# xxayt/MGSV

Measured on AMD Instinct MI355X. Metric: video-music pairs/s fwd+bwd at B=64 (full training step); sub-objects: retrieval sim-matrix GB/s, eval forward pairs/s, higher is better.
Workload: dtype bf16; 1 GPU; BASELINE.json configs[2]: B=64/GPU, T_v=30, T_a=512, D=512, train mode (dropout on), f32 master weights + Adam, f32 gradient accumulation; global_batch=64, launch=tape

## Files before the change

### include/made_hip.h

```cpp
#ifndef MADE_HIP_H
#define MADE_HIP_H

#include <stdint.h>

#ifdef __cplusplus
extern "C" {
#endif

#define MADE_ABI_VERSION 8

enum MadeDtype { MADE_F32 = 0, MADE_BF16 = 1 };

enum MadeAct {
    MADE_ACT_NONE = 0,
    MADE_ACT_RELU = 1,
    MADE_ACT_GELU = 2,
    MADE_ACT_QUICKGELU = 3,
    MADE_ACT_SIGMOID = 4
};

enum MadeGate {
    MADE_GATE_NONE = 0,
    MADE_GATE_RELU_OUT = 1,
    MADE_GATE_GELU_Z = 2,
// ... 629 lines not shown
} MadeResampleDesc;

int made_audio_resample(const float* pcm, int64_t pcm_len, const MadeResampleDesc* desc, int64_t n_tracks, const float* taps,
                        int64_t n_taps, float* out, int64_t out_len, void* stream);

typedef struct MadeAudioSegDesc {
    int64_t first;
    int64_t count;
} MadeAudioSegDesc;

int made_audio_fbank(const float* pcm, int64_t pcm_len, const MadeAudioSegDesc* segs, int64_t n_segs, const float* window,
                     const float* twiddle, const float* mel, int32_t mel_ld, float* spec, void* stream);

int made_ast_patches(const float* spec, int64_t n_segs, void* patches, int32_t patch_dtype, int64_t ld_patch, void* stream);

#ifdef __cplusplus
}
#endif
#endif
```

### mgsv_amd/_lib.py

```python
from __future__ import annotations

import ctypes as C
import os

_HERE = os.path.dirname(os.path.abspath(__file__))


def variant_env(name: str, default: str = "") -> str:
    if os.environ.get("MADE_DEBUG_VARIANTS", "0") in ("", "0"):
        return default
    return os.environ.get(name, default)


LIB_PATH = os.environ.get("MADE_LIB_PATH") or os.path.join(_HERE, "libmade_hip.so")
ABI_VERSION = 8

F32, BF16 = 0, 1
ACT_NONE, ACT_RELU, ACT_GELU, ACT_QUICKGELU, ACT_SIGMOID = 0, 1, 2, 3, 4
GATE_NONE, GATE_RELU_OUT, GATE_GELU_Z, GATE_QUICKGELU_Z, GATE_SIGMOID_OUT = 0, 1, 2, 3, 4

vp, i64, i32, f32 = C.c_void_p, C.c_int64, C.c_int32, C.c_float

WIDE_PLAN_HEAD, WIDE_PLAN_SAMPLE, WIDE_PLAN_SLOT, WIDE_PLAN_SLOT_BITS = 4, 4, 16, 8

# ... 169 lines not shown
                ("dtype", i32), ("_pad", i32)]


class MadeFrameDesc(C.Structure):
    _fields_ = [("offset", i64), ("coef", i64), ("H", i32), ("W", i32), ("kh", i32), ("kv", i32)]


class MadeResampleDesc(C.Structure):
    _fields_ = [("offset", i64), ("n", i64), ("taps", i64), ("o", i32), ("m", i32), ("width", i32), ("_pad", i32)]


class MadeAudioSegDesc(C.Structure):
    _fields_ = [("first", i64), ("count", i64)]


SIGNATURES = {
    "made_abi_version": (C.c_int, []),
    "made_set_f32_products": (C.c_int, [C.c_int]),
    "made_get_f32_products": (C.c_int, []),
    "made_last_error": (C.c_char_p, []),
    "made_device_info": (C.c_int, [C.c_char_p, C.c_int, C.POINTER(C.c_int), C.POINTER(C.c_int)]),
    "made_tape_begin": (C.c_int, []),
    "made_tape_end": (C.c_int, [C.POINTER(C.c_uint64)]),
    "made_tape_replay": (C.c_int, [C.c_uint64]),
    "made_tape_free": (C.c_int, [C.c_uint64]),
    "made_tape_interleave": (C.c_int, [C.c_uint64, i32]),
    "made_tape_count": (C.c_int, [C.c_uint64, C.POINTER(i64), C.POINTER(i64), C.POINTER(i64)]),
    "made_tape_replay_range": (C.c_int, [C.c_uint64, i64, i64]),
    "made_tape_op": (C.c_int, [C.c_uint64, i64, C.POINTER(i32), C.POINTER(C.c_uint64), C.POINTER(C.c_uint64), C.POINTER(C.c_uint32)]),
    "made_stream_wait": (C.c_int, [vp, vp]),
    "made_tape_event": (C.c_int, [i32, i32, vp]),
# ... 150 lines not shown
```

### mgsv_amd/ops_train.py

```python
from __future__ import annotations

import ctypes as C
from typing import Optional, Tuple

import torch

from . import _lib
from ._lib import BF16, F32, MadeAttnBwdArgs, MadeDropout, MadeGemmTNArgs, MadeGemmTNGroup, check, lib
from .ops import _f32, _p, _stream, _timed, dt_of, set_drop

Tensor = torch.Tensor
Pair = Tuple[int, int]


_TN_WS_LIMIT = 1 << 32
_TN_SLAB_US = 1.3


def _tn_splits(tiles: int, nslab: int, gathered: bool, cap: int) -> int:
    if _lib.variant_env("MADE_TN_SPLIT_MODEL", "1") == "0":
        sp = max(8, (512 // max(tiles, 1)) // 8 * 8) if cap == 64 and tiles < 64 else max(1, 2048 // max(tiles, 1))
        while (nslab + sp - 1) // sp > 64:
            sp += 8
        return min(sp, max(1, nslab))
    live = max(1, (nslab * 9) // 16 if gathered else nslab)
    best, best_t = 1, float("inf")
    for sp in (1, 2, 3, 4, 6, 8, 16, 24, 32, 40, 48, 56, 64):
# ... 242 lines not shown
    check(lib().made_pool_bwd(_p(_f32(mean, "mean")), _p(_f32(dvec, "dvec")), _p(_f32(mask, "mask")),
                              _p(in1), _dt(in1), *bs(in1), _p(in2), _dt(in2), *bs(in2),
                              _p(out), dt_of(out), *bs(out), B, T, D, eps, _stream()), "made_pool_bwd")
    return out


def l2norm_bwd(x: Tensor, dy: Tensor, dx: Optional[Tensor] = None, *, accumulate: bool = False, dx_alt: Optional[Tensor] = None,
               eps: float = 1e-12, dy_rows_per: int = 1) -> None:
    rows, D = x.shape
    check(lib().made_l2norm_bwd(_p(x), dt_of(x), x.stride(0), _p(_f32(dy, "dy")), dy.stride(0), dy_rows_per,
                                _p(dx), dx.stride(0) if dx is not None else 0, int(accumulate),
                                _p(dx_alt), _dt(dx_alt), dx_alt.stride(0) if dx_alt is not None else 0,
                                rows, D, eps, _stream()), "made_l2norm_bwd")


def clip_loss_bwd(sims: Tensor, logit_scale: Tensor, weight: float, upstream: Optional[Tensor], lse_ws: Tensor, dsims: Tensor,
                  dsims_t: Optional[Tensor], d_logit_scale: Optional[Tensor], accumulate: bool = False,
                  row_exclude: Optional[Tensor] = None) -> None:
    n = sims.shape[0]
    assert lse_ws.numel() >= 2 * n and dsims.is_contiguous()
    assert row_exclude is None or (row_exclude.shape == sims.shape and row_exclude.is_contiguous())
    check(lib().made_clip_loss_bwd(_p(_f32(sims, "sims")), sims.stride(0), n, _p(logit_scale), float(weight), _p(upstream),
                                   _p(lse_ws), _p(dsims), _p(dsims_t), int(accumulate), _p(d_logit_scale),
                                   _p(_f32(row_exclude, "row_exclude")), _stream()),
          "made_clip_loss_bwd")


def xpool_tail_bwd(y: Tensor, gamma: Tensor, beta: Tensor, video: Tensor, dsims: Tensor, dy: Tensor, Nm: int, Nv: int, *,
                   dy_drop: Optional[Tensor] = None, drop=None, dgamma: Optional[Tensor] = None, dbeta: Optional[Tensor] = None,
                   dvideo: Optional[Tensor] = None, dpool: Optional[Tensor] = None, dpool_scale: float = 1.0, eps: float = 1e-5) -> None:
# ... 122 lines not shown
```

### mgsv_amd/trainer.py

```python
from __future__ import annotations

import math
import os
from typing import Dict, List, Optional, Tuple

import numpy as np
import torch

from . import _lib, dropout as dr, ops, ops_train as tr, tape as _tape
from .config import MadeConfig
from .engine import MadeEngine
from .ops import Seg, round_up

WIDE_SLICES = 8

Tensor = torch.Tensor
XA = "video_guided_to_music_pooling_cross_transformer"


HEAD_PAD = 64


class MadeTrainer(MadeEngine):
    def __init__(self, cfg: MadeConfig, state_dict: Dict[str, object], device="cuda:0", dtype: str = "f32"):
# ... 499 lines not shown
        side.wait_stream(cur)
        self._index_lists(sm, tw["rows_a"], tw["order_a"])
        with torch.cuda.stream(side):
            self._fused_lists_fwd(ws, tw)
            self._encode_train(self._inputs[0], fm, "video", ws, tw, 0)
        self._encode_train(self._inputs[1], sm, "audio", ws, tw, Tv)
        cur.wait_stream(side)
        if "concat" in c.mml_fusion:
            frame, seg = ws["fus"][:, :Tv], ws["fus"][:, Tv:]
        else:
            frame, seg = ws["frame_buf"], ws["seg_buf"]
            self._ca_fusion_train(ws, tw, frame, seg, fm, sm, B, Tv, Ta)
        self._views = (frame, seg)
        out: Dict[str, Tensor] = dict(video_feats=ws["video"], music_feats=ws["music"], frame_feats=frame, segment_feats=seg)

        dec_early = None
        side.wait_stream(cur)
        with torch.cuda.stream(side):
            if getattr(self, "_zero_grad_in_forward", False):
                _tape.zero_(self.flat_grad)
                self._grads_zeroed = True
            if c.num_moment_queries == 1 and not regression and not xq and c.detr_enc_layers > 0:
                self._dec_fill_tgt(ws, tw)
                self._dec_query_side(tw, 0)
                dec_early = torch.cuda.Event()
                dec_early.record(side)
            out.update(self._retrieval_fwd(ws, tw, music_ids))
        out["memory"] = self._detr_encoder_fwd(ws, tw)
        if regression:
            out.update(self._regression_train(ws, tw, v_duration))
        else:
            if dec_early is not None:
                cur.wait_event(dec_early)
            else:
                if xq:
                    cur.wait_stream(side)
                self._dec_fill_tgt(ws, tw)
                self._dec_query_side(tw, 0)
            out.update(self._decoder_fwd(ws, tw))
            out.update(self._heads_fwd(ws, tw, v_duration))
        cur.wait_stream(side)
        return out
# ... 211 lines not shown
                h = ops.dec_stage(tb, P[p + ".ff1.w"], P[p + ".ff1.b"], tw[d + ".h"], ln=(P[p + ".ln2.g"], P[p + ".ln2.b"]), x_out=tw[d + ".t2"],
                                  act=ops.ACT_RELU, drop=self._drop(f"dec.{l}" + ".ffn_act", pd))
                t2 = tw[d + ".t2"]
            else:
                t2 = ops.layernorm(tb, P[p + ".ln2.g"], P[p + ".ln2.b"], out=tw[d + ".t2"])
                h = ops.linear(t2, P[p + ".ff1.w"], P[p + ".ff1.b"], act=ops.ACT_RELU, out=tw[d + ".h"], drop=self._drop(f"dec.{l}" + ".ffn_act", pd))
            tcx = ops.linear(h, P[p + ".ff2.w"], P[p + ".ff2.b"], R=t2, out=tw[d + ".t_c"], drop=self._drop(f"dec.{l}" + ".drop3", pd))
            t3 = tw[d + ".t3"]
            if stage:
                if l + 1 == nd:
                    ops.layernorm(tcx, P[p + ".ln3.g"], P[p + ".ln3.b"], out=t3)
            elif l + 1 < nd:
                ops.layernorm_add(tcx, P[p + ".ln3.g"], P[p + ".ln3.b"], self._query_pos_rows(), t3, tw[f"d.{l + 1}.tq"])
            else:
                ops.layernorm(tcx, P[p + ".ln3.g"], P[p + ".ln3.b"], out=t3)
        ops.layernorm(tw["dstack"]["tgt"][1:].reshape(nd * B * Q, D), P["dec.norm.g"], P["dec.norm.b"], out=hs.view(nd * B * Q, D))
        return dict(hs=hs.view(nd, B, Q, D))

    def _heads_fwd(self, ws, tw, v_duration: Optional[Tensor]) -> Dict[str, Tensor]:
        c, P = self.cfg, self.P
        B, Tv, _ = self._shape
        D, Q, nd = c.D, c.num_moment_queries, c.detr_dec_layers
        hs, music, frame = ws["hs"], ws["music"], self._views[0]
        out: Dict[str, Tensor] = {}
        hs2 = hs.view(nd * B * Q, D)
        logits, spans = ws["logits"], ws["spans"]
        ops.linear(hs2, P["class_embed.w"], P["class_embed.b"], out=logits.view(-1, 2))
        h1 = ops.linear(hs2, P["span_embed.0.w"], P["span_embed.0.b"], act=ops.ACT_RELU, out=tw["h1"])
        h2 = ops.linear(h1, P["span_embed.1.w"], P["span_embed.1.b"], act=ops.ACT_RELU, out=tw["h2"])
        if c.predict_center == 1:
            ops.linear(h2, P["span_embed.2.w"], P["span_embed.2.b"], act=ops.ACT_SIGMOID, segs=[Seg(out=spans.view(-1, 2), ldo=2)])
            spans[..., 1] = (v_duration.to(self.device, torch.float32) / c.max_m_duration).view(1, B, 1)
        else:
            ops.linear(h2, P["span_embed.2.w"], P["span_embed.2.b"], act=ops.ACT_SIGMOID, out=spans.view(-1, 2))
        out.update(pred_logits=logits[-1], pred_spans=spans[-1], logits_all=logits, spans_all=spans)
        if c.moment_loss:
            last = hs[nd - 1]
            m1 = ops.linear(last, P["moment_embed.0.w"], P["moment_embed.0.b"], act=ops.ACT_RELU)
            m2 = ops.linear(m1, P["moment_embed.1.w"], P["moment_embed.1.b"], act=ops.ACT_RELU)
            m3 = ops.linear(m2, P["moment_embed.2.w"], P["moment_embed.2.b"], out_dtype=torch.float32)
            mf = ops.l2norm_rows(m3)
            if c.audio_short_cut:
                mq = music if Q == 1 else music[:, None, :].expand(B, Q, D).contiguous()
                tr.add3(m3, mf, mq, b_mod=B * Q * D)
                mf = ops.l2norm_rows(m3)
            out["moment_feats"] = mf.view(B, Q, D)
        pq = vid_sum = None
        if c.contrastive_align_loss:
            ops.linear(hs2, P["proj_q.w"], P["proj_q.b"], out=ws["pq_raw"])
            pq = ws["pq"]
            pq2 = pq.view(nd * B * Q, -1)
            if c.audio_short_cut:
                mq = music if Q == 1 else music[:, None, :].expand(B, Q, D).contiguous()
                ops.l2norm_rows(ws["pq_raw"], out_f32=tw["pq_n0"])
                tr.add3(tw["pq_s1"], tw["pq_n0"], mq, b_mod=B * Q * D)
                ops.l2norm_rows(tw["pq_s1"], out_f32=pq2)
                if c.aux_loss and nd > 1:
                    n_aux = (nd - 1) * B * Q
                    tr.add3(tw["pq_s2"][:n_aux], pq2[:n_aux], mq, b_mod=B * Q * D)
                    ops.l2norm_rows(tw["pq_s2"][:n_aux], out_f32=pq2[:n_aux])
            else:
                ops.l2norm_rows(ws["pq_raw"], out_f32=pq2)
            self._frame_rows_linear(frame, P["proj_v.w"], P["proj_v.b"], ws["pv_raw"], B, Tv)
            pv = ws["pv"]
            ops.l2norm_rows(ws["pv_raw"], out_f32=pv.view(B * Tv, pq.shape[-1]))
            vid_sum = ops.masked_mean(pv, None, out=ws["vid_sum"])
            out.update(proj_queries=pq[-1], proj_vid_mem=pv, proj_queries_all=pq)
        tg = self._inputs[4]
        pi, ti, cnt, status, cost = ops.hungarian_match(logits.view(nd * B, Q, 2), spans.view(nd * B, Q, 2), tg, c.foreground_label)
        losses, total = ops.set_criterion(logits, spans, tg, pi, ti, cnt, pq, vid_sum, P["empty_weight"], c.foreground_label, P["crit_weights"])
        self._match = (pi, ti, cnt)
        out.update(matcher_pred_idx=pi.view(nd, B, -1), matcher_tgt_idx=ti.view(nd, B, -1), matcher_count=cnt.view(nd, B),
                   matcher_status=status, criterion_losses=losses, localization_loss=total)
        return out

    def _opt_stream(self):
        st = getattr(self, "_opt_st", None)
        if st is None:
            st = self._opt_st = torch.cuda.Stream(device=self.device)
        return st

    def _wide_slots(self) -> int:
        if getattr(self, "_wide_slots_n", None) is None:
            self._wide_slots_n = max(8, min(1024, _lib.device_info()[1]))
        return self._wide_slots_n

    def _wide_planned_ok(self, B: int, HQ: int, D: int) -> bool:
        return self.tc == torch.bfloat16 and D in (256, 512) and HQ <= 32 and B <= self._wide_slots()

    def _wide_split(self, B: int, backward: bool = False):
        plan = self._wide_plan
        if backward and self.cfg.detr_nheads * self.cfg.num_moment_queries > 8:
            plan = None
        if plan is not None:
            return WIDE_SLICES, plan
        return max(1, min(8, 256 // max(B, 1))), None

    def _dec_stage_chain(self) -> bool:
        c = self.cfg
        return (self.tc == torch.bfloat16 and c.num_moment_queries == 1 and c.D in (256, 512) and not c.detr_pre_norm
                and _lib.variant_env("MADE_DEC_STAGE", "1") != "0")

    def _encode_train(self, feats: Tensor, mask: Tensor, which: str, ws, tw, row_off: int) -> None:
        c, P = self.cfg, self.P
        if c.agg_module == "mlp":
            return self._encode_train_mlp(feats, mask, which, ws, tw, row_off)
        B, T, Kin = feats.shape
        D, Hh = c.D, c.SA_temporal_heads
        proj, mod, pe, depth, tag = (("vit_proj", "video_transformer", "pe_video", c.video_transformer_depth, "v") if which == "video"
                                     else ("ast_proj", "audio_transformer", "pe_audio", c.audio_transformer_depth, "a"))
        cls = bool(c.with_cls_token)
# ... 255 lines not shown
    def _heads_bwd(self, ws, tw, g_loc: Optional[Tensor]) -> list:
        c, P, G = self.cfg, self.P, self.G
        B, Tv, _ = self._shape
        D, Q, nd = c.D, c.num_moment_queries, c.detr_dec_layers
        tg, frame, dmusic = self._inputs[4], self._views[0], tw["dmusic"]
        logits, spans = ws["logits"], ws["spans"]
        pi, ti, cnt = self._match
        pq = ws["pq"] if c.contrastive_align_loss else None
        vid_sum = ws["vid_sum"] if c.contrastive_align_loss else None
        tr.set_criterion_bwd(logits, spans, tg, pi, ti, cnt, pq, vid_sum, P["empty_weight"], c.foreground_label, P["crit_weights"], g_loc,
                             tw["dlog"], tw["dsp"], tw["dpq"] if pq is not None else None, tw["dvid_sum"] if pq is not None else None,
                             ld_out=HEAD_PAD, through_sigmoid=True)
        hs2 = ws["hs"].view(nd * B * Q, D)
        dhs = tw["dhs"]
        dlog, dsp = tw["dlog"], tw["dsp"]
        if self.tc != torch.float32:
            tr.add3(tw["dlogsp_c"], tw["dlogsp"])
            dlog, dsp = tw["dlog_c"], tw["dsp_c"]
        heads_dw: list = []
        heads_dw.append(lambda: tr.gemm_tn(dlog[:, :2], hs2, G["class_embed.w"], accumulate=True, colsum=G["class_embed.b"]))
        ops.linear(dlog, P["class_embed.wt"], None, out=dhs)
        n_span = 1 if c.predict_center == 1 else 2
        heads_dw.append(lambda: tr.gemm_tn(dsp[:, :n_span], tw["h2"], G["span_embed.2.w"], accumulate=True, colsum=G["span_embed.2.b"]))
        dz2 = ops.linear(dsp, P["span_embed.2.wt"], None, out=tw["hg1"], gate=_lib.GATE_RELU_OUT, G=tw["h2"])
        dz1 = self._lin_bwd(dz2, tw["h1"], "span_embed.1", dx_out=tw["hg2"], gate=_lib.GATE_RELU_OUT, G=tw["h1"], later=heads_dw)
        self._lin_bwd(dz1, hs2, "span_embed.0", dx_out=dhs, R=dhs, later=heads_dw)
        if c.contrastive_align_loss:
            Dc = pq.shape[-1]
            dn = tw["dpq"]
            if c.audio_short_cut:
                if c.aux_loss and nd > 1:
                    n_aux = (nd - 1) * B * Q
                    ds2 = tw["dpq_s2"][:n_aux]
                    tr.l2norm_bwd(tw["pq_s2"][:n_aux], dn[:n_aux], dx=ds2)
                    dmusic.add_(ds2.view(nd - 1, B, Q, D).sum((0, 2)))
                    dn[:n_aux].copy_(ds2)
                tr.l2norm_bwd(tw["pq_s1"], dn, dx=tw["dpq_s"])
                dmusic.add_(tw["dpq_s"].view(nd, B, Q, D).sum((0, 2)))
                dn = tw["dpq_s"]
            tr.l2norm_bwd(ws["pq_raw"], dn, dx_alt=tw["dpq_raw"])
            self._lin_bwd(tw["dpq_raw"], hs2, "proj_q", dx_out=dhs, R=dhs, later=heads_dw)
            tr.l2norm_bwd(ws["pv_raw"], tw["dvid_sum"], dx_alt=tw["dpv_raw"], dy_rows_per=Tv)
            heads_dw.append(lambda: tr.gemm_tn(tw["dpv_raw"][:Tv], frame[0], G["proj_v.w"], accumulate=True, colsum=G["proj_v.b"], batch=(B, 1),
                                               a_zs=(Tv * Dc, 0), b_zs=(frame.stride(0), 0), colsum_zs=(0, 0)))
            ops.linear(tw["dpv_raw"], P["proj_v.wt"], None, out=tw["dframe_x"])
        return heads_dw

    def _fused_len(self) -> int:
        _, Tv, Ta = self._shape
        return Tv + Ta if "concat" in self.cfg.mml_fusion else Ta

    def _dec_self_attn_bwd(self, tw, l: int, g_sa: Tensor, gqkv: Tensor, g4: Tensor, dx_out: Tensor, R: Optional[Tensor] = None) -> Tensor:
        c, P, G = self.cfg, self.P, self.G
        B, D, Q, H = self._shape[0], c.D, c.num_moment_queries, c.detr_nheads
        p, d = f"detr_transformer.decoder.layers.{l}", f"d.{l}"
        datt = ops.linear(g_sa, P[p + ".sa.out.wt"], None, out=g4)
        q3, g3v = tw[d + ".qkv"].view(B, Q, 3 * D), gqkv.view(B, Q, 3 * D)
        tr.attention_bwd(q3[:, :, :D], q3[:, :, D:2 * D], q3[:, :, 2 * D:], tw[d + ".att"].view(B, Q, D), datt.view(B, Q, D),
                         g3v[:, :, :D], g3v[:, :, D:2 * D], g3v[:, :, 2 * D:], tw[d + ".lse"], tw["d_delta"], H,
                         drop=self._drop(f"dec.{l}" + ".sa_attn", float(c.detr_dropout)))
# ... 751 lines not shown
```

Baseline: 14150 pairs/s.

## Fuse DETR prediction heads into single forward and backward HIP kernels

Adds heads_fwd and heads_bwd kernels that fuse the decoder norm, class/span MLP, proj_q linear and L2 norm into one MFMA-based kernel per row tile. The backward kernel also fuses gradient casting, the first head linears and the L2-norm backward. By default it runs in the 'first' mode, where only the class/span-2 input grads come from the fused kernel. The frame-side proj_v path is moved off the critical chain, run on a separate event or deferred into the weight-gradient list. The aim is fewer small launches and less global memory traffic between them. The cost is new specialized kernels restricted to certain D and Dc configurations, plus extra complexity.

```diff
diff --git a/include/made_hip.h b/include/made_hip.h
--- a/include/made_hip.h
+++ b/include/made_hip.h
@@ -667,6 +667,36 @@
 
 int made_ast_patches(const float* spec, int64_t n_segs, void* patches, int32_t patch_dtype, int64_t ld_patch, void* stream);
 
+typedef struct MadeHeadsFwdArgs {
+    const void*  x;
+    const float* ln_g; const float* ln_b;
+    void*        hs;
+    const void*  Wc; const float* bc; float* logits;
+    const void*  W0; const float* b0; void* h1;
+    const void*  W1; const float* b1; void* h2;
+    const void*  W2; const float* b2; float* spans;
+    const void*  Wq; const float* bq; float* pq_raw; float* pq;
+    int64_t      rows, D, Dc;
+    float        ln_eps, l2_eps;
+    int32_t      predict_center; int32_t _pad;
+} MadeHeadsFwdArgs;
+int made_heads_fwd(const MadeHeadsFwdArgs* args, void* stream);
+
+typedef struct MadeHeadsBwdArgs {
+    const float* dlog; const float* dsp;
+    void*        dlog_c; void* dsp_c;
+    const void*  WcT; const void* W2T;
+    const void*  W1T; const void* W0T;
+    const void*  h1; const void* h2;
+    void*        hg1; void* hg2; void* dhs;
+    const float* pq_raw; const float* dpq;
+    void*        dpq_raw; const void* WqT;
+    int64_t      rows, D, Dc;
+    float        l2_eps;
+    int32_t      first_only;
+} MadeHeadsBwdArgs;
+int made_heads_bwd(const MadeHeadsBwdArgs* args, void* stream);
+
 #ifdef __cplusplus
 }
 #endif
diff --git a/mgsv_amd/_lib.py b/mgsv_amd/_lib.py
--- a/mgsv_amd/_lib.py
+++ b/mgsv_amd/_lib.py
@@ -207,7 +207,22 @@
     _fields_ = [("first", i64), ("count", i64)]
 
 
+class MadeHeadsFwdArgs(C.Structure):
+    _fields_ = [("x", vp), ("ln_g", vp), ("ln_b", vp), ("hs", vp),
+                ("Wc", vp), ("bc", vp), ("logits", vp), ("W0", vp), ("b0", vp), ("h1", vp), ("W1", vp), ("b1", vp), ("h2", vp),
+                ("W2", vp), ("b2", vp), ("spans", vp), ("Wq", vp), ("bq", vp), ("pq_raw", vp), ("pq", vp),
+                ("rows", i64), ("D", i64), ("Dc", i64), ("ln_eps", f32), ("l2_eps", f32), ("predict_center", i32), ("_pad", i32)]
+
+
+class MadeHeadsBwdArgs(C.Structure):
+    _fields_ = [("dlog", vp), ("dsp", vp), ("dlog_c", vp), ("dsp_c", vp), ("WcT", vp), ("W2T", vp), ("W1T", vp), ("W0T", vp),
+                ("h1", vp), ("h2", vp), ("hg1", vp), ("hg2", vp), ("dhs", vp), ("pq_raw", vp), ("dpq", vp), ("dpq_raw", vp), ("WqT", vp),
+                ("rows", i64), ("D", i64), ("Dc", i64), ("l2_eps", f32), ("first_only", i32)]
+
+
 SIGNATURES = {
+    "made_heads_fwd": (C.c_int, [C.POINTER(MadeHeadsFwdArgs), vp]),
+    "made_heads_bwd": (C.c_int, [C.POINTER(MadeHeadsBwdArgs), vp]),
     "made_abi_version": (C.c_int, []),
     "made_set_f32_products": (C.c_int, [C.c_int]),
     "made_get_f32_products": (C.c_int, []),
diff --git a/mgsv_amd/csrc/heads.hip b/mgsv_amd/csrc/heads.hip
--- /dev/null
+++ b/mgsv_amd/csrc/heads.hip
@@ -0,0 +1,408 @@
+#include "common.h"
+
+namespace {
+
+constexpr int H_ROWS = 16, H_THREADS = 512, H_WAVES = H_THREADS / WAVE;
+constexpr int H_PAD = 8;
+constexpr int H_HEAD = 64;
+constexpr int H_DC_MAX = 256;
+
+__device__ __forceinline__ int live_row(int e, int hh) { return (e & 3) + 8 * (e >> 2) + 4 * hh; }
+
+template <int SPQ>
+__device__ __forceinline__ void tile_product(const bf16_t* __restrict__ pw, const bf16_t* sa, float* v) {
+    bf16x8 fw[4 * SPQ];
+#pragma unroll
+    for (int s = 0; s < 4 * SPQ; ++s) fw[s] = *(const bf16x8*)(pw + s * 16);
+    f32x16 acc[4];
+#pragma unroll
+    for (int q = 0; q < 4; ++q) {
+#pragma unroll
+        for (int e = 0; e < 16; ++e) acc[q][e] = 0.f;
+#pragma unroll
+        for (int s = 0; s < SPQ; ++s) {
+            const bf16x8 fa = *(const bf16x8*)(sa + (q * SPQ + s) * 16);
+            acc[q] = __builtin_amdgcn_mfma_f32_32x32x16_bf16(fa, fw[q * SPQ + s], acc[q], 0, 0, 0);
+        }
+    }
+#pragma unroll
+    for (int e = 0; e < 8; ++e) {
+        v[e] = 0.f;
+#pragma unroll
+        for (int q = 0; q < 4; ++q) v[e] += acc[q][e];
+    }
+}
+
+template <int SPQ> constexpr int W_RS = SPQ * 16 + 8;
+__device__ __forceinline__ void wave_lds_handover() {
+    asm volatile("" ::: "memory");
+    __builtin_amdgcn_wave_barrier();
+    asm volatile("" ::: "memory");
+}
+template <int SPQ>
+__device__ __forceinline__ void tile_product_staged(const bf16_t* __restrict__ W, int n0, int N, bf16_t* sw, const bf16_t* sa, float* v) {
+    static_assert(SPQ == 4 || SPQ == 8, "staged tiles: K = 256 or 512");
+    constexpr int K = 64 * SPQ, RS = W_RS<SPQ>, LPR = 2 * SPQ, RPI = 64 / LPR;
+    const int lane = threadIdx.x & 63, r = lane & 31, hh = lane >> 5;
+    const int lrow = lane / LPR, lchunk = lane % LPR;
+    bf16x8 fw[4 * SPQ];
+#pragma unroll
+    for (int q = 0; q < 4; ++q)
+#pragma unroll
+        for (int i = 0; i < SPQ; ++i) {
+            int n = n0 + i * RPI + lrow; n = n < N ? n : N - 1;
+            fw[q * SPQ + i] = *(const bf16x8*)(W + (int64_t)n * K + q * (K / 4) + lchunk * 8);
+        }
+    f32x16 acc[4];
+#pragma unroll
+    for (int q = 0; q < 4; ++q) {
+        wave_lds_handover();
+#pragma unroll
+        for (int i = 0; i < SPQ; ++i) *(bf16x8*)(sw + (i * RPI + lrow) * RS + lchunk * 8) = fw[q * SPQ + i];
+        wave_lds_handover();
+#pragma unroll
+        for (int e = 0; e < 16; ++e) acc[q][e] = 0.f;
+#pragma unroll
+        for (int s = 0; s < SPQ; ++s) {
+            const bf16x8 fa = *(const bf16x8*)(sa + (q * SPQ + s) * 16);
+            const bf16x8 fb = *(const bf16x8*)(sw + r * RS + s * 16 + hh * 8);
+            acc[q] = __builtin_amdgcn_mfma_f32_32x32x16_bf16(fa, fb, acc[q], 0, 0, 0);
+        }
+    }
+#pragma unroll
+    for (int e = 0; e < 8; ++e) {
+        v[e] = 0.f;
+#pragma unroll
+        for (int q = 0; q < 4; ++q) v[e] += acc[q][e];
+    }
+}
+
+__device__ __forceinline__ void tile_product_k(int spq, const bf16_t* __restrict__ pw, const bf16_t* sa, float* v) {
+    switch (spq) {
+        case 1: tile_product<1>(pw, sa, v); break;
+        case 2: tile_product<2>(pw, sa, v); break;
+        default: tile_product<4>(pw, sa, v); break;
+    }
+}
+
+__device__ __forceinline__ void copy_rows_out(const bf16_t* s, int ld, bf16_t* g, int D, int64_t m0, int64_t rows) {
+    const int per = D / 8;
+    for (int i = threadIdx.x; i < H_ROWS * per; i += H_THREADS) {
+        const int row = i / per, c = (i - row * per) * 8;
+        if (m0 + row < rows) *(bf16x8*)(g + (m0 + row) * D + c) = *(const bf16x8*)(s + row * ld + c);
+    }
+}
+
+template <int D>
+__global__ __launch_bounds__(H_THREADS) void heads_fwd_kernel(const MadeHeadsFwdArgs a) {
+    constexpr int LD = D + H_PAD, SPQ = D / 64, NT = D / 32;
+    __shared__ __attribute__((aligned(16))) bf16_t sX[2][H_ROWS * LD];
+    __shared__ __attribute__((aligned(16))) float sP[H_ROWS * H_DC_MAX];
+    extern __shared__ __attribute__((aligned(16))) unsigned char heads_dyn[];
+    const int tid = threadIdx.x, lane = tid & 63, wave = tid >> 6;
+    bf16_t* sw = (bf16_t*)heads_dyn + wave * (32 * W_RS<SPQ>);
+    const int r = lane & 31, hh = lane >> 5;
+    const int64_t rows = a.rows, m0 = (int64_t)blockIdx.x * H_ROWS;
+    const int Dc = (int)a.Dc;
+
+#pragma unroll
+    for (int rr = 0; rr < H_ROWS / H_WAVES; ++rr) {
+        const int lr = wave * (H_ROWS / H_WAVES) + rr;
+        const int64_t gm = m0 + lr, gmc = gm < rows ? gm : rows - 1;
+        const bf16_t* x = (const bf16_t*)a.x + gmc * D;
+        f32x4 v[2];
+        float sum = 0.f;
+#pragma unroll
+        for (int i = 0; i < 2; ++i) {
+            const int c = (i * WAVE + lane) * 4;
+            if (c < D) {
+                const bf16x4 t = *(const bf16x4*)(x + c);
+                v[i][0] = (float)t[0]; v[i][1] = (float)t[1]; v[i][2] = (float)t[2]; v[i][3] = (float)t[3];
+                sum += (v[i][0] + v[i][1]) + (v[i][2] + v[i][3]);
+            }
+        }
+        const float mean = wave_sum(sum) / (float)D;
+        float sq = 0.f;
+#pragma unroll
+        for (int i = 0; i < 2; ++i) {
+            const int c = (i * WAVE + lane) * 4;
+            if (c < D) {
+#pragma unroll
+                for (int j = 0; j < 4; ++j) { float d = v[i][j] - mean; sq += d * d; }
+            }
+        }
+        const float rstd = 1.0f / sqrtf(wave_sum(sq) / (float)D + a.ln_eps);
+#pragma unroll
+        for (int i = 0; i < 2; ++i) {
+            const int c = (i * WAVE + lane) * 4;
+            if (c < D) {
+                const f32x4 g = *(const f32x4*)(a.ln_g + c), bb = *(const f32x4*)(a.ln_b + c);
+                f32x4 o;
+#pragma unroll
+                for (int j = 0; j < 4; ++j) o[j] = (v[i][j] - mean) * rstd * g[j] + bb[j];
+                bf16x4 t;
+                t[0] = (bf16_t)o[0]; t[1] = (bf16_t)o[1]; t[2] = (bf16_t)o[2]; t[3] = (bf16_t)o[3];
+                *(bf16x4*)(sX[0] + lr * LD + c) = t;
+                if (gm < rows) *(bf16x4*)((bf16_t*)a.hs + gm * D + c) = t;
+            }
+        }
+    }
+    __syncthreads();
+
+    const bf16_t* sa0 = sX[0] + (r & 15) * LD + hh * 8;
+    const bf16_t* sa1 = sX[1] + (r & 15) * LD + hh * 8;
+
+    const int ntq = (Dc + 31) / 32;
+    for (int t = wave; t < NT + ntq + 1; t += H_WAVES) {
+        const int kind = t < NT ? 0 : (t < NT + ntq ? 1 : 2);
+        const int n0 = kind == 0 ? t * 32 : (kind == 1 ? (t - NT) * 32 : 0);
+        const int N = kind == 0 ? D : (kind == 1 ? Dc : 2);
+        const bf16_t* W = (const bf16_t*)(kind == 0 ? a.W0 : (kind == 1 ? a.Wq : a.Wc));
+        const float* bias = kind == 0 ? a.b0 : (kind == 1 ? a.bq : a.bc);
+        const int n = n0 + r, nc = n < N ? n : N - 1;
+        const float bv = bias[nc];
+        float v[8];
+        tile_product_staged<SPQ>(W, n0, N, sw, sa0, v);
+#pragma unroll
+        for (int e = 0; e < 8; ++e) {
+            const int lr = live_row(e, hh);
+            const int64_t gm = m0 + lr;
+            float o = v[e] + bv;
+            if (kind == 0) {
+                sX[1][lr * LD + n] = (bf16_t)fmaxf(o, 0.f);
+            } else if (kind == 1) {
+                if (n < N) {
+                    sP[lr * H_DC_MAX + n] = o;
+                    if (gm < rows) a.pq_raw[gm * Dc + n] = o;
+                }
+            } else if (n < 2 && gm < rows) {
+                a.logits[gm * 2 + n] = o;
+            }
+        }
+    }
+    __syncthreads();
+
+    for (int t = wave; t < NT; t += H_WAVES) {
+        const int n = t * 32 + r;
+        const float bv = a.b1[n];
+        float v[8];
+        tile_product_staged<SPQ>((const bf16_t*)a.W1, t * 32, D, sw, sa1, v);
+#pragma unroll
+        for (int e = 0; e < 8; ++e) sX[0][live_row(e, hh) * LD + n] = (bf16_t)fmaxf(v[e] + bv, 0.f);
+    }
+    if (Dc > 0) {
+#pragma unroll
+        for (int rr = 0; rr < H_ROWS / H_WAVES; ++rr) {
+            const int lr = wave * (H_ROWS / H_WAVES) + rr;
+            const int64_t gm = m0 + lr;
+            const int c = lane * 4;
+            f32x4 v;
+            float sq = 0.f;
+            if (c < Dc) {
+                v = *(const f32x4*)(sP + lr * H_DC_MAX + c);
+#pragma unroll
+                for (int j = 0; j < 4; ++j) sq += v[j] * v[j];
+            }
+            const float nrm = fmaxf(sqrtf(wave_sum(sq)), a.l2_eps);
+            if (c < Dc && gm < rows) {
+                f32x4 o;
+#pragma unroll
+                for (int j = 0; j < 4; ++j) o[j] = v[j] / nrm;
+                *(f32x4*)(a.pq + gm * Dc + c) = o;
+            }
+        }
+    }
+    __syncthreads();
+
+    if (wave == 0) {
+        const int nc = r < 2 ? r : 1;
+        const float bv = a.b2[nc];
+        float v[8];
+        tile_product_staged<SPQ>((const bf16_t*)a.W2, 0, 2, sw, sa0, v);
+        const int ncol = a.predict_center ? 1 : 2;
+#pragma unroll
+        for (int e = 0; e < 8; ++e) {
+            const int64_t gm = m0 + live_row(e, hh);
+            const float x = v[e] + bv;
+            const float o = 1.f / (1.f + expf(-x));
+            if (r < ncol && gm < rows) a.spans[gm * 2 + r] = o;
+        }
+    }
+    copy_rows_out(sX[1], LD, (bf16_t*)a.h1, D, m0, rows);
+    copy_rows_out(sX[0], LD, (bf16_t*)a.h2, D, m0, rows);
+}
+
+template <int D>
+__global__ __launch_bounds__(H_THREADS) void heads_bwd_kernel(const MadeHeadsBwdArgs a) {
+    constexpr int LD = D + H_PAD, SPQ = D / 64, NT = D / 32, OWN = NT / H_WAVES, LDG = H_HEAD + H_PAD, LDQ = H_DC_MAX + H_PAD;
+    __shared__ __attribute__((aligned(16))) bf16_t sX[3][H_ROWS * LD];
+    __shared__ __attribute__((aligned(16))) bf16_t sG[2][H_ROWS * LDG];
+    __shared__ __attribute__((aligned(16))) bf16_t sQ[H_ROWS * LDQ];
+    extern __shared__ __attribute__((aligned(16))) unsigned char heads_dyn[];
+    const int tid = threadIdx.x, lane = tid & 63, wave = tid >> 6;
+    bf16_t* sw = (bf16_t*)heads_dyn + wave * (32 * W_RS<SPQ>);
+    const int r = lane & 31, hh = lane >> 5;
+    const int64_t rows = a.rows, m0 = (int64_t)blockIdx.x * H_ROWS;
+    const int Dc = (int)a.Dc;
+
+    {
+        const int which = tid >> 8, lr = (tid >> 4) & 15, c = (tid & 15) * 4;
+        const int64_t gm = m0 + lr, gmc = gm < rows ? gm : rows - 1;
+        const f32x4 g = *(const f32x4*)((which ? a.dsp : a.dlog) + gmc * H_HEAD + c);
+        bf16x4 t;
+        t[0] = (bf16_t)g[0]; t[1] = (bf16_t)g[1]; t[2] = (bf16_t)g[2]; t[3] = (bf16_t)g[3];
+        *(bf16x4*)(sG[which] + lr * LDG + c) = t;
+        if (gm < rows) *(bf16x4*)((bf16_t*)(which ? a.dsp_c : a.dlog_c) + gm * H_HEAD + c) = t;
+    }
+    if (Dc > 0) {
+#pragma unroll
+        for (int rr = 0; rr < H_ROWS / H_WAVES; ++rr) {
+            const int lr = wave * (H_ROWS / H_WAVES) + rr;
+            const int64_t gm = m0 + lr, gmc = gm < rows ? gm : rows - 1;
+            const int c = lane * 4, cc = c < Dc ? c : 0;
+            f32x4 xv = *(const f32x4*)(a.pq_raw + gmc * Dc + cc), gv = *(const f32x4*)(a.dpq + gmc * Dc + cc);
+            if (c >= Dc) {
+#pragma unroll
+                for (int j = 0; j < 4; ++j) { xv[j] = 0.f; gv[j] = 0.f; }
+            }
+            float nn = 0.f, dot = 0.f;
+#pragma unroll
+            for (int j = 0; j < 4; ++j) { nn += xv[j] * xv[j]; dot += xv[j] * gv[j]; }
+            const float nrm = fmaxf(sqrtf(wave_sum(nn)), a.l2_eps);
+            dot = wave_sum(dot) / (nrm * nrm);
+            if (c < Dc) {
+                f32x4 o;
+#pragma unroll
+                for (int j = 0; j < 4; ++j) o[j] = (gv[j] - xv[j] * dot) / nrm;
+                bf16x4 t;
+                t[0] = (bf16_t)o[0]; t[1] = (bf16_t)o[1]; t[2] = (bf16_t)o[2]; t[3] = (bf16_t)o[3];
+                *(bf16x4*)(sQ + lr * LDQ + c) = t;
+                if (gm < rows) *(bf16x4*)((bf16_t*)a.dpq_raw + gm * Dc + c) = t;
+            }
+        }
+    }
+    __syncthreads();
+
+    float dhs[OWN][8];
+    int64_t grow[8];
+#pragma unroll
+    for (int e = 0; e < 8; ++e) { const int64_t gm = m0 + live_row(e, hh); grow[e] = gm < rows ? gm : rows - 1; }
+
+#pragma unroll
+    for (int o = 0; o < OWN; ++o) {
+        const int n = (wave + o * H_WAVES) * 32 + r;
+        bf16_t gate[8];
+#pragma unroll
+        for (int e = 0; e < 8; ++e) gate[e] = ((const bf16_t*)a.h2)[grow[e] * D + n];
+        float v[8];
+        tile_product<1>((const bf16_t*)a.WcT + (int64_t)n * H_HEAD + hh * 8, sG[0] + (r & 15) * LDG + hh * 8, v);
+#pragma unroll
+        for (int e = 0; e < 8; ++e) dhs[o][e] = (float)(bf16_t)(v[e] + 0.f);
+        tile_product<1>((const bf16_t*)a.W2T + (int64_t)n * H_HEAD + hh * 8, sG[1] + (r & 15) * LDG + hh * 8, v);
+#pragma unroll
+        for (int e = 0; e < 8; ++e) {
+            float x = v[e] + 0.f;
+            x *= ((float)gate[e] != 0.f ? 1.f : 0.f) * 1.f;
+            sX[0][live_row(e, hh) * LD + n] = (bf16_t)x;
+        }
+        if (a.first_only) {
+#pragma unroll
+            for (int e = 0; e < 8; ++e) sX[2][live_row(e, hh) * LD + n] = (bf16_t)dhs[o][e];
+        }
+    }
+    __syncthreads();
+    if (a.first_only) {
+        copy_rows_out(sX[0], LD, (bf16_t*)a.hg1, D, m0, rows);
+        copy_rows_out(sX[2], LD, (bf16_t*)a.dhs, D, m0, rows);
+        return;
+    }
+
+#pragma unroll
+    for (int o = 0; o < OWN; ++o) {
+        const int n = (wave + o * H_WAVES) * 32 + r;
+        bf16_t gate[8];
+#pragma unroll
+        for (int e = 0; e < 8; ++e) gate[e] = ((const bf16_t*)a.h1)[grow[e] * D + n];
+        float v[8];
+        tile_product_staged<SPQ>((const bf16_t*)a.W1T, (wave + o * H_WAVES) * 32, D, sw, sX[0] + (r & 15) * LD + hh * 8, v);
+#pragma unroll
+        for (int e = 0; e < 8; ++e) {
+            float x = v[e] + 0.f;
+            x *= ((float)gate[e] != 0.f ? 1.f : 0.f) * 1.f;
+            sX[1][live_row(e, hh) * LD + n] = (bf16_t)x;
+        }
+    }
+    __syncthreads();
+
+#pragma unroll
+    for (int o = 0; o < OWN; ++o) {
+        const int n = (wave + o * H_WAVES) * 32 + r;
+        float v[8];
+        tile_product_staged<SPQ>((const bf16_t*)a.W0T, (wave + o * H_WAVES) * 32, D, sw, sX[1] + (r & 15) * LD + hh * 8, v);
+#pragma unroll
+        for (int e = 0; e < 8; ++e) dhs[o][e] = (float)(bf16_t)((v[e] + 0.f) + dhs[o][e]);
+        if (Dc > 0) {
+            tile_product_k(Dc / 64, (const bf16_t*)a.WqT + (int64_t)n * Dc + hh * 8, sQ + (r & 15) * LDQ + hh * 8, v);
+#pragma unroll
+            for (int e = 0; e < 8; ++e) dhs[o][e] = (float)(bf16_t)((v[e] + 0.f) + dhs[o][e]);
+        }
+#pragma unroll
+        for (int e = 0; e < 8; ++e) sX[2][live_row(e, hh) * LD + n] = (bf16_t)dhs[o][e];
+    }
+    __syncthreads();
+    copy_rows_out(sX[0], LD, (bf16_t*)a.hg1, D, m0, rows);
+    copy_rows_out(sX[1], LD, (bf16_t*)a.hg2, D, m0, rows);
+    copy_rows_out(sX[2], LD, (bf16_t*)a.dhs, D, m0, rows);
+}
+
+bool aligned16(const void* p) { return ((uintptr_t)p & 15) == 0; }
+
+constexpr unsigned slab_bytes(int D) { return (unsigned)(H_WAVES * 32 * (D / 4 + 8) * sizeof(bf16_t)); }
+
+template <typename Kern> bool allow_slabs(Kern k, int D) {
+    return hipFuncSetAttribute((const void*)k, hipFuncAttributeMaxDynamicSharedMemorySize, (int)slab_bytes(D)) == hipSuccess;
+}
+
+}
+
+extern "C" int made_heads_fwd(const MadeHeadsFwdArgs* args, void* stream) {
+    MADE_REQUIRE(args != nullptr, "made_heads_fwd: null args");
+    const MadeHeadsFwdArgs& a = *args;
+    MADE_REQUIRE(a.x && a.ln_g && a.ln_b && a.hs && a.Wc && a.bc && a.logits && a.W0 && a.b0 && a.h1 && a.W1 && a.b1 && a.h2 &&
+                 a.W2 && a.b2 && a.spans, "made_heads_fwd: null pointer");
+    MADE_REQUIRE(a.rows >= 0, "made_heads_fwd: negative rows");
+    MADE_UNSUPPORTED(a.D == 256 || a.D == 512, "made_heads_fwd: D=%lld must be 256 or 512", (long long)a.D);
+    MADE_UNSUPPORTED(a.Dc == 0 || a.Dc == 64 || a.Dc == 128 || a.Dc == 256, "made_heads_fwd: Dc=%lld must be 0, 64, 128 or 256", (long long)a.Dc);
+    if (a.Dc > 0) MADE_REQUIRE(a.Wq && a.bq && a.pq_raw && a.pq, "made_heads_fwd: Dc > 0 needs Wq, bq, pq_raw and pq");
+    MADE_UNSUPPORTED(aligned16(a.x) && aligned16(a.hs) && aligned16(a.h1) && aligned16(a.h2) && aligned16(a.Wc) && aligned16(a.W0) &&
+                     aligned16(a.W1) && aligned16(a.W2) && aligned16(a.Wq) && aligned16(a.pq) && aligned16(a.ln_g) && aligned16(a.ln_b),
+                     "made_heads_fwd: rows must be 16-byte aligned");
+    if (a.rows == 0) return MADE_OK;
+    const dim3 grid((unsigned)((a.rows + H_ROWS - 1) / H_ROWS)), block(H_THREADS);
+    static const bool once = allow_slabs(heads_fwd_kernel<512>, 512) && allow_slabs(heads_fwd_kernel<256>, 256);
+    MADE_REQUIRE(once, "made_heads_fwd: hipFuncSetAttribute(MaxDynamicSharedMemorySize) failed");
+    if (a.D == 512) hipLaunchKernelGGL((heads_fwd_kernel<512>), grid, block, slab_bytes(512), (hipStream_t)stream, a);
+    else hipLaunchKernelGGL((heads_fwd_kernel<256>), grid, block, slab_bytes(256), (hipStream_t)stream, a);
+    return made_check_launch("made_heads_fwd");
+}
+
+extern "C" int made_heads_bwd(const MadeHeadsBwdArgs* args, void* stream) {
+    MADE_REQUIRE(args != nullptr, "made_heads_bwd: null args");
+    const MadeHeadsBwdArgs& a = *args;
+    MADE_REQUIRE(a.dlog && a.dsp && a.dlog_c && a.dsp_c && a.WcT && a.W2T && a.h2 && a.hg1 && a.dhs, "made_heads_bwd: null pointer");
+    MADE_REQUIRE(a.first_only || (a.W1T && a.W0T && a.h1 && a.hg2), "made_heads_bwd: the whole chain needs W1T, W0T, h1 and hg2");
+    MADE_REQUIRE(a.rows >= 0, "made_heads_bwd: negative rows");
+    MADE_UNSUPPORTED(a.D == 256 || a.D == 512, "made_heads_bwd: D=%lld must be 256 or 512", (long long)a.D);
+    MADE_UNSUPPORTED(a.Dc == 0 || a.Dc == 64 || a.Dc == 128 || a.Dc == 256, "made_heads_bwd: Dc=%lld must be 0, 64, 128 or 256", (long long)a.Dc);
+    if (a.Dc > 0) MADE_REQUIRE(a.pq_raw && a.dpq && a.dpq_raw && (a.first_only || a.WqT), "made_heads_bwd: Dc > 0 needs pq_raw, dpq, dpq_raw and WqT");
+    MADE_UNSUPPORTED(aligned16(a.dlog) && aligned16(a.dsp) && aligned16(a.dlog_c) && aligned16(a.dsp_c) && aligned16(a.WcT) && aligned16(a.W2T) &&
+                     aligned16(a.W1T) && aligned16(a.W0T) && aligned16(a.hg1) && aligned16(a.hg2) && aligned16(a.dhs) && aligned16(a.pq_raw) &&
+                     aligned16(a.dpq) && aligned16(a.dpq_raw) && aligned16(a.WqT), "made_heads_bwd: rows must be 16-byte aligned");
+    if (a.rows == 0) return MADE_OK;
+    const dim3 grid((unsigned)((a.rows + H_ROWS - 1) / H_ROWS)), block(H_THREADS);
+    static const bool once = allow_slabs(heads_bwd_kernel<512>, 512) && allow_slabs(heads_bwd_kernel<256>, 256);
+    MADE_REQUIRE(once, "made_heads_bwd: hipFuncSetAttribute(MaxDynamicSharedMemorySize) failed");
+    if (a.D == 512) hipLaunchKernelGGL((heads_bwd_kernel<512>), grid, block, slab_bytes(512), (hipStream_t)stream, a);
+    else hipLaunchKernelGGL((heads_bwd_kernel<256>), grid, block, slab_bytes(256), (hipStream_t)stream, a);
+    return made_check_launch("made_heads_bwd");
+}
diff --git a/mgsv_amd/ops_train.py b/mgsv_amd/ops_train.py
--- a/mgsv_amd/ops_train.py
+++ b/mgsv_amd/ops_train.py
@@ -11,6 +11,7 @@
 
 Tensor = torch.Tensor
 Pair = Tuple[int, int]
+TPair = Tuple[Tensor, Tensor]
 
 
 _TN_WS_LIMIT = 1 << 32
@@ -283,6 +284,61 @@
                                 rows, D, eps, _stream()), "made_l2norm_bwd")
 
 
+def _rows_of(t: Tensor, dtype, rows: int, cols: int, name: str) -> Tensor:
+    if t.dtype != dtype or tuple(t.shape) != (rows, cols) or not t.is_contiguous():
+        raise TypeError(f"{name} must be a contiguous {dtype} tensor of shape ({rows}, {cols}), got {t.dtype} {tuple(t.shape)}")
+    return t
+
+
+def heads_fwd(x: Tensor, ln: TPair, hs: Tensor, cls: TPair, logits: Tensor, span0: TPair, h1: Tensor, span1: TPair, h2: Tensor,
+              span2: TPair, spans: Tensor, proj: Optional[TPair] = None, pq_raw: Optional[Tensor] = None, pq: Optional[Tensor] = None,
+              *, predict_center: bool = False, ln_eps: float = 1e-5, l2_eps: float = 1e-12) -> None:
+    bf, f = torch.bfloat16, torch.float32
+    rows, D = x.shape
+    a = _lib.MadeHeadsFwdArgs()
+    a.x, a.hs = _p(_rows_of(x, bf, rows, D, "x")), _p(_rows_of(hs, bf, rows, D, "hs"))
+    a.ln_g, a.ln_b = _p(_f32(ln[0], "ln.g")), _p(_f32(ln[1], "ln.b"))
+    a.Wc, a.bc, a.logits = _p(_rows_of(cls[0], bf, 2, D, "cls.w")), _p(_f32(cls[1], "cls.b")), _p(_rows_of(logits, f, rows, 2, "logits"))
+    a.W0, a.b0, a.h1 = _p(_rows_of(span0[0], bf, D, D, "span0.w")), _p(_f32(span0[1], "span0.b")), _p(_rows_of(h1, bf, rows, D, "h1"))
+    a.W1, a.b1, a.h2 = _p(_rows_of(span1[0], bf, D, D, "span1.w")), _p(_f32(span1[1], "span1.b")), _p(_rows_of(h2, bf, rows, D, "h2"))
+    a.W2, a.b2, a.spans = _p(_rows_of(span2[0], bf, 2, D, "span2.w")), _p(_f32(span2[1], "span2.b")), _p(_rows_of(spans, f, rows, 2, "spans"))
+    Dc = 0
+    if proj is not None:
+        Dc = proj[0].shape[0]
+        a.Wq, a.bq = _p(_rows_of(proj[0], bf, Dc, D, "proj.w")), _p(_f32(proj[1], "proj.b"))
+        a.pq_raw, a.pq = _p(_rows_of(pq_raw, f, rows, Dc, "pq_raw")), _p(_rows_of(pq, f, rows, Dc, "pq"))
+    a.rows, a.D, a.Dc, a.ln_eps, a.l2_eps, a.predict_center = rows, D, Dc, ln_eps, l2_eps, int(bool(predict_center))
+    _timed("heads_fwd_kernel", 2.0 * rows * D * (2 * D + Dc + 4), float(((rows + 15) // 16) * 2 * D * (2 * D + Dc + 4) + 4 * rows * D * 2),
+           lambda: check(lib().made_heads_fwd(C.byref(a), _stream()), "made_heads_fwd"), f"rows={rows} D={D} Dc={Dc}")
+
+
+def heads_bwd(dlog: Tensor, dsp: Tensor, dlog_c: Tensor, dsp_c: Tensor, cls_wt: Tensor, span2_wt: Tensor, span1_wt: Optional[Tensor],
+              span0_wt: Optional[Tensor], h1: Optional[Tensor], h2: Tensor, hg1: Tensor, hg2: Optional[Tensor], dhs: Tensor,
+              pq_raw: Optional[Tensor] = None, dpq: Optional[Tensor] = None, dpq_raw: Optional[Tensor] = None,
+              proj_wt: Optional[Tensor] = None, *, first_only: bool = False, l2_eps: float = 1e-12) -> None:
+    bf, f = torch.bfloat16, torch.float32
+    rows, D = h2.shape
+    a = _lib.MadeHeadsBwdArgs()
+    a.dlog, a.dsp = _p(_rows_of(dlog, f, rows, 64, "dlog")), _p(_rows_of(dsp, f, rows, 64, "dsp"))
+    a.dlog_c, a.dsp_c = _p(_rows_of(dlog_c, bf, rows, 64, "dlog_c")), _p(_rows_of(dsp_c, bf, rows, 64, "dsp_c"))
+    a.WcT, a.W2T = _p(_rows_of(cls_wt, bf, D, 64, "cls_wt")), _p(_rows_of(span2_wt, bf, D, 64, "span2_wt"))
+    if not first_only:
+        a.W1T, a.W0T = _p(_rows_of(span1_wt, bf, D, D, "span1_wt")), _p(_rows_of(span0_wt, bf, D, D, "span0_wt"))
+        a.h1, a.hg2 = _p(_rows_of(h1, bf, rows, D, "h1")), _p(_rows_of(hg2, bf, rows, D, "hg2"))
+    a.h2 = _p(_rows_of(h2, bf, rows, D, "h2"))
+    a.hg1, a.dhs = _p(_rows_of(hg1, bf, rows, D, "hg1")), _p(_rows_of(dhs, bf, rows, D, "dhs"))
+    Dc = 0
+    if pq_raw is not None:
+        Dc = pq_raw.shape[1]
+        if not first_only:
+            a.WqT = _p(_rows_of(proj_wt, bf, D, Dc, "proj_wt"))
+        a.pq_raw, a.dpq = _p(_rows_of(pq_raw, f, rows, Dc, "pq_raw")), _p(_rows_of(dpq, f, rows, Dc, "dpq"))
+        a.dpq_raw = _p(_rows_of(dpq_raw, bf, rows, Dc, "dpq_raw"))
+    a.rows, a.D, a.Dc, a.l2_eps, a.first_only = rows, D, Dc, l2_eps, int(bool(first_only))
+    _timed("heads_bwd_kernel", 2.0 * rows * D * (2 * D + Dc + 128), float(((rows + 15) // 16) * 2 * D * (2 * D + Dc + 128) + 5 * rows * D * 2),
+           lambda: check(lib().made_heads_bwd(C.byref(a), _stream()), "made_heads_bwd"), f"rows={rows} D={D} Dc={Dc}")
+
+
 def clip_loss_bwd(sims: Tensor, logit_scale: Tensor, weight: float, upstream: Optional[Tensor], lse_ws: Tensor, dsims: Tensor,
                   dsims_t: Optional[Tensor], d_logit_scale: Optional[Tensor], accumulate: bool = False,
                   row_exclude: Optional[Tensor] = None) -> None:
diff --git a/mgsv_amd/trainer.py b/mgsv_amd/trainer.py
--- a/mgsv_amd/trainer.py
+++ b/mgsv_amd/trainer.py
@@ -537,7 +537,7 @@
         self._views = (frame, seg)
         out: Dict[str, Tensor] = dict(video_feats=ws["video"], music_feats=ws["music"], frame_feats=frame, segment_feats=seg)
 
-        dec_early = None
+        dec_early = self._frames_done = None
         side.wait_stream(cur)
         with torch.cuda.stream(side):
             if getattr(self, "_zero_grad_in_forward", False):
@@ -549,6 +549,10 @@
                 dec_early = torch.cuda.Event()
                 dec_early.record(side)
             out.update(self._retrieval_fwd(ws, tw, music_ids))
+            if c.contrastive_align_loss and not regression and self._frame_side_off_chain():
+                self._frame_side_fwd(ws)
+                self._frames_done = torch.cuda.Event()
+                self._frames_done.record(side)
         out["memory"] = self._detr_encoder_fwd(ws, tw)
         if regression:
             out.update(self._regression_train(ws, tw, v_duration))
@@ -790,7 +794,8 @@
                 ops.layernorm_add(tcx, P[p + ".ln3.g"], P[p + ".ln3.b"], self._query_pos_rows(), t3, tw[f"d.{l + 1}.tq"])
             else:
                 ops.layernorm(tcx, P[p + ".ln3.g"], P[p + ".ln3.b"], out=t3)
-        ops.layernorm(tw["dstack"]["tgt"][1:].reshape(nd * B * Q, D), P["dec.norm.g"], P["dec.norm.b"], out=hs.view(nd * B * Q, D))
+        if self._heads_fused() != "full":
+            ops.layernorm(tw["dstack"]["tgt"][1:].reshape(nd * B * Q, D), P["dec.norm.g"], P["dec.norm.b"], out=hs.view(nd * B * Q, D))
         return dict(hs=hs.view(nd, B, Q, D))
 
     def _heads_fwd(self, ws, tw, v_duration: Optional[Tensor]) -> Dict[str, Tensor]:
@@ -801,14 +806,24 @@
         out: Dict[str, Tensor] = {}
         hs2 = hs.view(nd * B * Q, D)
         logits, spans = ws["logits"], ws["spans"]
-        ops.linear(hs2, P["class_embed.w"], P["class_embed.b"], out=logits.view(-1, 2))
-        h1 = ops.linear(hs2, P["span_embed.0.w"], P["span_embed.0.b"], act=ops.ACT_RELU, out=tw["h1"])
-        h2 = ops.linear(h1, P["span_embed.1.w"], P["span_embed.1.b"], act=ops.ACT_RELU, out=tw["h2"])
+        fused = self._heads_fused() == "full"
+        if fused:
+            cal = bool(c.contrastive_align_loss)
+            tr.heads_fwd(tw["dstack"]["tgt"][1:].reshape(nd * B * Q, D), (P["dec.norm.g"], P["dec.norm.b"]), hs2,
+                         (P["class_embed.w"], P["class_embed.b"]), logits.view(-1, 2), (P["span_embed.0.w"], P["span_embed.0.b"]), tw["h1"],
+                         (P["span_embed.1.w"], P["span_embed.1.b"]), tw["h2"], (P["span_embed.2.w"], P["span_embed.2.b"]), spans.view(-1, 2),
+                         (P["proj_q.w"], P["proj_q.b"]) if cal else None, ws["pq_raw"] if cal else None,
+                         ws["pq"].view(nd * B * Q, -1) if cal else None, predict_center=c.predict_center == 1)
+        else:
+            ops.linear(hs2, P["class_embed.w"], P["class_embed.b"], out=logits.view(-1, 2))
+            h1 = ops.linear(hs2, P["span_embed.0.w"], P["span_embed.0.b"], act=ops.ACT_RELU, out=tw["h1"])
+            h2 = ops.linear(h1, P["span_embed.1.w"], P["span_embed.1.b"], act=ops.ACT_RELU, out=tw["h2"])
+            if c.predict_center == 1:
+                ops.linear(h2, P["span_embed.2.w"], P["span_embed.2.b"], act=ops.ACT_SIGMOID, segs=[Seg(out=spans.view(-1, 2), ldo=2)])
+            else:
+                ops.linear(h2, P["span_embed.2.w"], P["span_embed.2.b"], act=ops.ACT_SIGMOID, out=spans.view(-1, 2))
         if c.predict_center == 1:
-            ops.linear(h2, P["span_embed.2.w"], P["span_embed.2.b"], act=ops.ACT_SIGMOID, segs=[Seg(out=spans.view(-1, 2), ldo=2)])
             spans[..., 1] = (v_duration.to(self.device, torch.float32) / c.max_m_duration).view(1, B, 1)
-        else:
-            ops.linear(h2, P["span_embed.2.w"], P["span_embed.2.b"], act=ops.ACT_SIGMOID, out=spans.view(-1, 2))
         out.update(pred_logits=logits[-1], pred_spans=spans[-1], logits_all=logits, spans_all=spans)
         if c.moment_loss:
             last = hs[nd - 1]
@@ -823,10 +838,13 @@
             out["moment_feats"] = mf.view(B, Q, D)
         pq = vid_sum = None
         if c.contrastive_align_loss:
-            ops.linear(hs2, P["proj_q.w"], P["proj_q.b"], out=ws["pq_raw"])
+            if not fused:
+                ops.linear(hs2, P["proj_q.w"], P["proj_q.b"], out=ws["pq_raw"])
             pq = ws["pq"]
             pq2 = pq.view(nd * B * Q, -1)
-            if c.audio_short_cut:
+            if fused:
+                pass
+            elif c.audio_short_cut:
                 mq = music if Q == 1 else music[:, None, :].expand(B, Q, D).contiguous()
                 ops.l2norm_rows(ws["pq_raw"], out_f32=tw["pq_n0"])
                 tr.add3(tw["pq_s1"], tw["pq_n0"], mq, b_mod=B * Q * D)
@@ -837,10 +855,11 @@
                     ops.l2norm_rows(tw["pq_s2"][:n_aux], out_f32=pq2[:n_aux])
             else:
                 ops.l2norm_rows(ws["pq_raw"], out_f32=pq2)
-            self._frame_rows_linear(frame, P["proj_v.w"], P["proj_v.b"], ws["pv_raw"], B, Tv)
-            pv = ws["pv"]
-            ops.l2norm_rows(ws["pv_raw"], out_f32=pv.view(B * Tv, pq.shape[-1]))
-            vid_sum = ops.masked_mean(pv, None, out=ws["vid_sum"])
+            if self._frames_done is None:
+                self._frame_side_fwd(ws)
+            else:
+                torch.cuda.current_stream().wait_event(self._frames_done)
+            pv, vid_sum = ws["pv"], ws["vid_sum"]
             out.update(proj_queries=pq[-1], proj_vid_mem=pv, proj_queries_all=pq)
         tg = self._inputs[4]
         pi, ti, cnt, status, cost = ops.hungarian_match(logits.view(nd * B, Q, 2), spans.view(nd * B, Q, 2), tg, c.foreground_label)
@@ -850,6 +869,16 @@
                    matcher_status=status, criterion_losses=losses, localization_loss=total)
         return out
 
+    def _frame_side_fwd(self, ws) -> None:
+        P = self.P
+        B, Tv, _ = self._shape
+        self._frame_rows_linear(self._views[0], P["proj_v.w"], P["proj_v.b"], ws["pv_raw"], B, Tv)
+        ops.l2norm_rows(ws["pv_raw"], out_f32=ws["pv"].view(B * Tv, -1))
+        ops.masked_mean(ws["pv"], None, out=ws["vid_sum"])
+
+    def _frame_side_off_chain(self) -> bool:
+        return _lib.variant_env("MADE_HEADS_FUSED", "1") != "0"
+
     def _opt_stream(self):
         st = getattr(self, "_opt_st", None)
         if st is None:
@@ -871,6 +900,14 @@
         if plan is not None:
             return WIDE_SLICES, plan
         return max(1, min(8, 256 // max(B, 1))), None
+
+    def _heads_fused(self) -> str:
+        c = self.cfg
+        knob = _lib.variant_env("MADE_HEADS_FUSED", "1")
+        if not (self.tc == torch.bfloat16 and c.D in (256, 512) and not c.detr_pre_norm and not c.audio_short_cut and not c.moment_loss
+                and (not c.contrastive_align_loss or c.contrastive_hdim in (64, 128, 256))) or knob == "0":
+            return ""
+        return "full" if knob == "full" else "first"
 
     def _dec_stage_chain(self) -> bool:
         c = self.cfg
@@ -1156,17 +1193,29 @@
         hs2 = ws["hs"].view(nd * B * Q, D)
         dhs = tw["dhs"]
         dlog, dsp = tw["dlog"], tw["dsp"]
-        if self.tc != torch.float32:
+        mode = self._heads_fused()
+        fused, first = mode == "full", mode != ""
+        if first:
+            cal = bool(c.contrastive_align_loss)
+            tr.heads_bwd(dlog, dsp, tw["dlog_c"], tw["dsp_c"], P["class_embed.wt"], P["span_embed.2.wt"],
+                         P["span_embed.1.wt"] if fused else None, P["span_embed.0.wt"] if fused else None, tw["h1"] if fused else None,
+                         tw["h2"], tw["hg1"], tw["hg2"] if fused else None, dhs, ws["pq_raw"] if cal else None,
+                         tw["dpq"] if cal else None, tw["dpq_raw"] if cal else None, P["proj_q.wt"] if (cal and fused) else None,
+                         first_only=not fused)
+            dlog, dsp = tw["dlog_c"], tw["dsp_c"]
+        elif self.tc != torch.float32:
             tr.add3(tw["dlogsp_c"], tw["dlogsp"])
             dlog, dsp = tw["dlog_c"], tw["dsp_c"]
         heads_dw: list = []
         heads_dw.append(lambda: tr.gemm_tn(dlog[:, :2], hs2, G["class_embed.w"], accumulate=True, colsum=G["class_embed.b"]))
-        ops.linear(dlog, P["class_embed.wt"], None, out=dhs)
+        if not first:
+            ops.linear(dlog, P["class_embed.wt"], None, out=dhs)
         n_span = 1 if c.predict_center == 1 else 2
         heads_dw.append(lambda: tr.gemm_tn(dsp[:, :n_span], tw["h2"], G["span_embed.2.w"], accumulate=True, colsum=G["span_embed.2.b"]))
-        dz2 = ops.linear(dsp, P["span_embed.2.wt"], None, out=tw["hg1"], gate=_lib.GATE_RELU_OUT, G=tw["h2"])
-        dz1 = self._lin_bwd(dz2, tw["h1"], "span_embed.1", dx_out=tw["hg2"], gate=_lib.GATE_RELU_OUT, G=tw["h1"], later=heads_dw)
-        self._lin_bwd(dz1, hs2, "span_embed.0", dx_out=dhs, R=dhs, later=heads_dw)
+        dz2 = tw["hg1"] if first else ops.linear(dsp, P["span_embed.2.wt"], None, out=tw["hg1"], gate=_lib.GATE_RELU_OUT, G=tw["h2"])
+        dz1 = tw["hg2"]
+        self._lin_bwd(dz2, tw["h1"], "span_embed.1", dx_out=None if fused else dz1, gate=_lib.GATE_RELU_OUT, G=tw["h1"], later=heads_dw)
+        self._lin_bwd(dz1, hs2, "span_embed.0", dx_out=None if fused else dhs, R=dhs, later=heads_dw)
         if c.contrastive_align_loss:
             Dc = pq.shape[-1]
             dn = tw["dpq"]
@@ -1180,12 +1229,18 @@
                 tr.l2norm_bwd(tw["pq_s1"], dn, dx=tw["dpq_s"])
                 dmusic.add_(tw["dpq_s"].view(nd, B, Q, D).sum((0, 2)))
                 dn = tw["dpq_s"]
-            tr.l2norm_bwd(ws["pq_raw"], dn, dx_alt=tw["dpq_raw"])
-            self._lin_bwd(tw["dpq_raw"], hs2, "proj_q", dx_out=dhs, R=dhs, later=heads_dw)
-            tr.l2norm_bwd(ws["pv_raw"], tw["dvid_sum"], dx_alt=tw["dpv_raw"], dy_rows_per=Tv)
+            if not first:
+                tr.l2norm_bwd(ws["pq_raw"], dn, dx_alt=tw["dpq_raw"])
+            self._lin_bwd(tw["dpq_raw"], hs2, "proj_q", dx_out=None if fused else dhs, R=dhs, later=heads_dw)
+            def frame_side():
+                tr.l2norm_bwd(ws["pv_raw"], tw["dvid_sum"], dx_alt=tw["dpv_raw"], dy_rows_per=Tv)
+                ops.linear(tw["dpv_raw"], P["proj_v.wt"], None, out=tw["dframe_x"])
+            if self._frame_side_off_chain():
+                heads_dw.insert(0, frame_side)
+            else:
+                frame_side()
             heads_dw.append(lambda: tr.gemm_tn(tw["dpv_raw"][:Tv], frame[0], G["proj_v.w"], accumulate=True, colsum=G["proj_v.b"], batch=(B, 1),
                                                a_zs=(Tv * Dc, 0), b_zs=(frame.stride(0), 0), colsum_zs=(0, 0)))
-            ops.linear(tw["dpv_raw"], P["proj_v.wt"], None, out=tw["dframe_x"])
         return heads_dw
 
     def _fused_len(self) -> int:
```

Measured after the change: 14250 pairs/s (median of 6 runs). Within noise of the previous version (+0.7%).
